# probcomp/GenParticleFilters.jl

Measured on AMD Instinct MI355X. Metric: particle-steps/sec, higher is better.
Workload: dtype f64; 1 GPU; 2D linear-Gaussian SSM, bootstrap PF, multinomial resample every step (BASELINE.json configs[1]); particles_per_gpu=1000000, particles_total=1000000, T=3059, state_dim=2, parallelism=particle-shard x1

## Files before the change

### genparticlefilters.jl_amd/csrc/gpf_host.hpp

```cpp
#pragma once
#include "../../include/gpf.h"
#include "gpf_kernels.hpp"

#include <hip/hip_ext.h>
#include <rccl/rccl.h>
#include <dlfcn.h>
#include <unistd.h>

#include <algorithm>
#include <cmath>
#include <cstdio>
#include <cstring>
#include <mutex>
#include <string>
#include <type_traits>
#include <vector>

using namespace gpf;

namespace gpfh {

static inline void cpu_relax()
{
#if defined(__x86_64__) || defined(__i386__)
// ... 54 lines not shown
    Scalars* sc = nullptr;
    Scalars* h_sc = nullptr;
    long long* h_sc_ticket = nullptr; long long sc_ticket = 0;
    uint32_t epoch = 0;
    bool initialized = false, has_prev = false, raw_valid = false, residual_scanned = false;
    bool max_valid = false;
    bool raw_sum_valid = false;
    WSum sum_cache{};
    uint64_t* sum_part = nullptr;
    int64_t* h_spart = nullptr;
    bool sum_on_host = false;
    uint64_t* gate_part = nullptr; int gate_cur = 0; int64_t* h_gate = nullptr;
    bool raw_has_q = false;
    bool raw_q_folded = false;
    bool pending_gather = false;
    bool pending_fill = false;
    bool pending_search = false;
    SearchArgs pend_sa{};
    bool pending_move = false; int pm_method = 0, pm_iters = 0; uint32_t pm_epoch = 0; ModelArgs pm_args{};
    bool lazy_move = true;
    bool lazy_search = false;
    bool want_offsets = true;
    bool ch0_offsets = false;
    bool offsets_hint = true;
    bool pending_packed = false;
    const double* pend_packed = nullptr; const double* pend_mf = nullptr; const int64_t* pend_tot = nullptr; int pend_G = 0;
    bool pend_mailbox = false;
    bool pend_own = false; int64_t pend_m = 0; bool pend_own_range = false;
    double* fuse_mf_out = nullptr;
    bool own_direct = false;
    bool own_direct_range = false;
    bool hist_on = false;
    int hist_cap = 0;
    std::vector<double*> hist_x;
    std::vector<int32_t*> hist_map;
    int hist_step = -1;
    const int32_t** hist_dev_maps = nullptr;
    gpf_filter* parent = nullptr;
    std::vector<gpf_filter*> views;
    bool orphaned = false;
    int64_t view_start = 0;
    int64_t view_step = 1;
    double* vrows[2] = {nullptr, nullptr}; double* vlw = nullptr; int32_t* vanc = nullptr;
    int32_t* vidx = nullptr; int32_t* vgid = nullptr;
    uint64_t generation = 0;
    uint64_t parent_generation = 0;
// ... 336 lines not shown
```

### genparticlefilters.jl_amd/csrc/gpf_k_scan.hpp

```cpp
#pragma once

namespace gpf {
static __global__ __launch_bounds__(BLOCK) void k_max_partial(PrioView pv, int64_t n, MaxSlots ms)
{
    double m = -__builtin_huge_val();
    int f = 0;
    for (int64_t i = (int64_t)blockIdx.x * BLOCK + threadIdx.x; i < n; i += (int64_t)gridDim.x * BLOCK) track_max(pv.at(i), m, f);
    block_max_store(m, f, ms);
}

constexpr uint64_t DESC_VALID = 1ull << 63, DESC_MASK = (1ull << 63) - 1;
constexpr unsigned SPIN_LIMIT = 1u << 22;

__device__ __forceinline__ void desc_store(uint64_t* p, uint64_t v)
{
    __hip_atomic_store(p, v, __ATOMIC_RELAXED, __HIP_MEMORY_SCOPE_AGENT);
}
__device__ __forceinline__ uint64_t desc_load(const uint64_t* p)
{
    return __hip_atomic_load(const_cast<uint64_t*>(p), __ATOMIC_RELAXED, __HIP_MEMORY_SCOPE_AGENT);
}
__device__ __forceinline__ uint64_t desc_wait(const uint64_t* p, int32_t* timeout)
{
    uint64_t d = desc_load(p);
// ... 104 lines not shown
};
#ifndef GPF_SCAN_BLOCK
#define GPF_SCAN_BLOCK 256
#endif
constexpr int SCAN_BLOCK = GPF_SCAN_BLOCK;
constexpr int SCAN_NWAVES = SCAN_BLOCK / WAVE;
constexpr int SCAN_ROWS = TILE / (2 * SCAN_BLOCK);
static_assert(SCAN_ROWS * 2 * SCAN_BLOCK == TILE && SCAN_ROWS >= 2 && SCAN_ROWS % 2 == 0, "a wave owns whole 256-element groups");
template <class In, int MODE>
__global__ __launch_bounds__(SCAN_BLOCK) void k_scan(In in, int64_t n, int64_t ntiles,
                                                const double* __restrict__ mf_all, const unsigned long long* __restrict__ slots,
                                                int np, WSum* __restrict__ ws_out, ScanOut out,
                                                uint64_t* __restrict__ dcur, uint64_t* __restrict__ dnext,
                                                uint64_t* __restrict__ total_out, uint64_t* __restrict__ blockQ,
                                                int32_t* __restrict__ timeout, ScanExtras ex)
{
    const unsigned G = gridDim.x - (unsigned)ex.sp.blocks;
    if (blockIdx.x >= G) { sorted_gamma_tile(ex.sp, (int64_t)(blockIdx.x - G) * SCAN_BLOCK + threadIdx.x); return; }
    if (ex.zero128 && blockIdx.x == 0)
        for (int i = threadIdx.x; i < 2 * MAX_SHARDS * ex.zero_stride; i += SCAN_BLOCK) ex.zero128[i] = 0;
    __shared__ uint64_t s_wave[SCAN_NWAVES];
    __shared__ uint64_t s_red[SCAN_NWAVES];
    __shared__ uint64_t s_Stot;
    uint64_t* const d_agg = dcur;
    uint64_t* const d_pre = dcur + ntiles;
    for (int64_t i = (int64_t)blockIdx.x * SCAN_BLOCK + threadIdx.x; i < 2 * ntiles; i += (int64_t)G * SCAN_BLOCK) dnext[i] = 0;
    constexpr bool WANT_Q = MODE == 2 || MODE == 4;
    double pre[2 * SCAN_ROWS];
    if constexpr (MODE >= 1) {
        const int64_t wb0 = (int64_t)blockIdx.x * TILE + (int64_t)wave_id() * (SCAN_ROWS * 2 * WAVE) + 2 * lane_id();
#pragma unroll
        for (int k = 0; k < SCAN_ROWS; ++k) in.raw2(wb0 + k * 2 * WAVE, n, pre[2 * k], pre[2 * k + 1]);
    }
    if constexpr (MODE >= 1) {
        double m; int f;
        if constexpr (MODE >= 3) {
            double m0 = 0.0; int f0 = 0;
            if (ex.fuse_mf) {
                fold_slots(slots, m0, f0);
                f0 &= FLAG_NAN | FLAG_POSINF;
                if (blockIdx.x == 0 && wave_id() == 0) {
                    if (lane_id() == 0) { ex.mf_out[0] = m0; ex.mf_out[1] = (double)f0; }
                    const uint64_t words[2] = {d2u(m0), d2u((double)f0)};
                    mbox_push_wave(ex.mf_push, words);
                }
            }
            mbox_wait_block(ex.wait);
            const int g = lane_id();
            const bool mb = ex.wait.tags != nullptr;
            const bool self = ex.fuse_mf && g == ex.mf_me;
            m = g < np ? (self ? m0 : ld_gathered(mf_all + 2 * g, mb)) : -__builtin_huge_val();
            f = g < np ? (self ? f0 : (int)ld_gathered(mf_all + 2 * g + 1, mb)) : 0;
            m = wave_max_f64(m);
#pragma unroll
            for (int s = 32; s >= 1; s >>= 1) f |= __shfl_xor(f, s, WAVE);
            if (!(f & FLAG_NAN) && m == -__builtin_huge_val()) f |= FLAG_ALL_NEGINF;
        } else fold_slots(slots, m, f);
        in.m = m; in.flags = f;
        if (blockIdx.x == 0 && threadIdx.x == 0) {
// ... 16 lines not shown
            uint64_t q0, q1;
            cb[k] = carry;
            if constexpr (MODE >= 1) {
                if (tile == blockIdx.x) in.conv2(wbase + k * 2 * WAVE, n, pre[2 * k], pre[2 * k + 1], q0, q1);
                else in.load2(wbase + k * 2 * WAVE, n, q0, q1);
            } else in.load2(wbase + k * 2 * WAVE, n, q0, q1);
            if constexpr (WANT_Q) {
                uint64_t lo = q0 * q0, hi = __umul64hi(q0, q0);
                ql[0] += lo & 0xffffffffull; ql[1] += lo >> 32; ql[2] += hi & 0xffffffffull; ql[3] += hi >> 32;
                lo = q1 * q1; hi = __umul64hi(q1, q1);
                ql[0] += lo & 0xffffffffull; ql[1] += lo >> 32; ql[2] += hi & 0xffffffffull; ql[3] += hi >> 32;
            }
            const uint64_t pair = q0 + q1;
            const uint64_t inc = wave_scan_u64(pair);
            p[2 * k] = carry + (inc - pair) + q0;
            p[2 * k + 1] = p[2 * k] + q1;
            carry += shfl_u64(inc, WAVE - 1);
        }
        if (lane == 0) s_wave[wv] = carry;
        __syncthreads();
        uint64_t wexcl = 0, agg = 0;
#pragma unroll
        for (int w = 0; w < SCAN_NWAVES; ++w) { if (w < wv) wexcl += s_wave[w]; agg += s_wave[w]; }
        if (threadIdx.x == 0) desc_store(d_agg + tile, DESC_VALID | agg);
        const int64_t first = (tile / G) * G;
        uint64_t acc = 0;
        for (int64_t idx = first + threadIdx.x; idx < tile; idx += SCAN_BLOCK) acc += desc_wait(d_agg + idx, timeout);
        if (first > 0 && threadIdx.x == SCAN_BLOCK - 1) acc += desc_wait(d_pre + first - 1, timeout);
        acc = wave_sum_u64(acc);
        if (lane == 0) s_red[wv] = acc;
        __syncthreads();
        uint64_t excl = 0;
#pragma unroll
        for (int w = 0; w < SCAN_NWAVES; ++w) excl += s_red[w];
        if (threadIdx.x == 0) desc_store(d_pre + tile, DESC_VALID | (excl + agg));
        const uint64_t off = excl + wexcl;
        if (out.cdf) {
#pragma unroll
            for (int k = 0; k < SCAN_ROWS; ++k) {
                const int64_t idx = wbase + k * 2 * WAVE;
                const uint64_t v1 = off + p[2 * k + 1];
                *reinterpret_cast<ulonglong2*>(out.cdf + idx) = make_ulonglong2(off + p[2 * k], v1);
                if ((lane & 7) == 7) out.t16[(idx + 1) >> 4] = v1;
                if ((lane & 15) == 15) out.k32[(idx + 1) >> 5] = (uint32_t)(key_sat(v1) >> KEY_SHIFT);
                if (lane == WAVE - 1 && (k & 1)) out.t256[(idx + 1) >> 8] = v1;
                if (out.k32s && lane == WAVE - 1) out.k32s[(idx + 1) >> 7] = (uint32_t)(key_sat(v1) >> KEY_SHIFT);
                if (out.off16) {
                    const int GL = 16 << out.logg;
                    const uint32_t kv = (uint32_t)(key_sat(v1) >> KEY_SHIFT);
                    const uint32_t khi = (uint32_t)__shfl((int)kv, lane | (GL - 1), WAVE);
                    const uint32_t kprev = (uint32_t)__shfl((int)kv, ((lane & ~(GL - 1)) - 1) & (WAVE - 1), WAVE);
                    const uint32_t klo = lane < GL ? (uint32_t)(key_sat(off + cb[k]) >> KEY_SHIFT) : kprev;
                    const int sh = key_quant_shift(klo, khi);
                    const uint64_t kb = (uint64_t)klo << KEY_SHIFT;
                    const uint32_t o0 = (uint32_t)((key_sat(off + p[2 * k]) - kb) >> sh), o1 = (uint32_t)((key_sat(v1) - kb) >> sh);
                    reinterpret_cast<uint32_t*>(out.off16)[idx >> 1] = o0 | (o1 << 16);
                    if (out.logg == 0) {
                        const uint32_t part = (uint32_t)__builtin_amdgcn_update_dpp(0, (int)o1, 0x55, 0xF, 0xF, false);
                        if ((lane & 3) == 3) reinterpret_cast<uint32_t*>(out.coarse)[(idx + 1) >> 3] = part | (o1 << 16);
                    } else {
                        const uint32_t part = (uint32_t)__builtin_amdgcn_update_dpp(0, (int)o1, 0x114, 0xF, 0xF, false);
                        if ((lane & 7) == 7) reinterpret_cast<uint32_t*>(out.coarse)[(idx + 1) >> 4] = part | (o1 << 16);
                    }
                }
            }
        }
        if constexpr (MODE == 3) {
            if (tile == ntiles - 1 && wv == SCAN_NWAVES - 1) {
                const uint64_t Sw = shfl_u64(off + p[2 * SCAN_ROWS - 1], WAVE - 1);
                const uint64_t words[5] = {Sw, 0, 0, 0, 0};
                mbox_push_wave(ex.push, words);
            }
        }
        if (tile == ntiles - 1 && threadIdx.x == SCAN_BLOCK - 1) {
            const uint64_t Stot = off + p[2 * SCAN_ROWS - 1];
            *total_out = Stot;
            if constexpr (WANT_Q) s_Stot = Stot;
            if constexpr (MODE >= 1) {
                if (ex.n_slots > 0) {
                    const uint64_t Bq = Stot / (uint64_t)ex.n_slots;
                    ws_out->sB = Bq; ws_out->srem = Stot - Bq * (uint64_t)ex.n_slots;
                    ws_out->sinv = (double)ex.n_slots / (double)Stot;
                }
            }
        }
        if constexpr (MODE == 3) {
            if (ex.splan.plan && tile == ntiles - 1) {
                static_assert(SCAN_BLOCK > MAX_SHARDS, "one thread per shard boundary");
                __shared__ int64_t s_F[MAX_SHARDS + 1];
                const StratPlanJob& jb = ex.splan;
                strat_plan_body(jb, [&](int g) { return shard_bound(jb.n_global, jb.G, g); }, s_F);
            }
        }
        __syncthreads();
    }
    if constexpr (WANT_Q) {
        __shared__ uint64_t s_q[SCAN_NWAVES][4];
// ... 522 lines not shown
```

### genparticlefilters.jl_amd/csrc/gpf_k_search.hpp

```cpp
#pragma once

namespace gpf {
struct CdfLevels {
    const uint64_t* cdf;  const uint64_t* t16;  const uint64_t* t256;  const uint64_t* ttile;
    const uint32_t* k32;
    const uint16_t* off16; const uint16_t* coarse; int logg;
    const uint32_t* k32s; int sample;
};
__device__ __forceinline__ ulonglong2 load_global_16(uint64_t addr, int sub)
{
#if defined(__HIP_DEVICE_COMPILE__)
    typedef unsigned long long __attribute__((ext_vector_type(2))) u64x2;
    const __attribute__((address_space(1))) u64x2* g = reinterpret_cast<const __attribute__((address_space(1))) u64x2*>(addr);
    const u64x2 v = g[sub];
    return make_ulonglong2(v.x, v.y);
#else
    (void)addr; (void)sub;
    return make_ulonglong2(0, 0);
#endif
}

__device__ __forceinline__ int group8_sum(int c)
{
    c += __builtin_amdgcn_update_dpp(0, c, 0xB1, 0xF, 0xF, false);
    c += __builtin_amdgcn_update_dpp(0, c, 0x4E, 0xF, 0xF, false);
    c += __builtin_amdgcn_update_dpp(0, c, 0x141, 0xF, 0xF, false);
    return c;
}
__device__ __forceinline__ void coop_count_le2(const uint64_t* line0, uint64_t T0, const uint64_t* line1, uint64_t T1,
                                               ulonglong2* lds_wave, int& c0, int& c1)
// ... 240 lines not shown
            head[u] = false; top[u] = st.topw; L[u] = &a.w;
            if (METHOD == 0) T[u] = mulhi64(U, S);
            else if (METHOD == 3) {
                T[u] = jg * s_div[0] + (jg * s_div[1] + mulhi64(U, S)) / N;
            } else {
                head[u] = jg < Ctot;
                T[u] = head[u] ? jg : mulhi64(U, S);
                if (head[u]) { top[u] = st.topc; L[u] = &a.c; }
            }
        }
        const bool coop = METHOD == 0 ? true : (METHOD == 3 ? false : __any(!head[0] || !head[1]) != 0);
        int64_t idx[2];
        search_pair(st, L, top, T, coop, lds_wave, a.n_cells, a.ntiles, idx);
#pragma unroll
        for (int u = 0; u < 2; ++u) {
            if (act[u]) a.anc[j[u]] = (int32_t)idx[u];
        }
    }
}

constexpr int MULTI_LDS_BUDGET = 160 * 1024 - 2048;
__host__ __device__ __forceinline__ int64_t multi_groups(int64_t ntiles, int logg) { return (ntiles * (TILE / 32)) >> logg; }
__host__ __device__ __forceinline__ uint32_t kpad(uint32_t i) { return i + (i >> 5); }
__host__ inline size_t multi_lds_bytes(int64_t ntiles, int logg) { return (size_t)(kpad((uint32_t)multi_groups(ntiles, logg)) + 1) * sizeof(uint32_t); }
#ifndef GPF_MULTI_MIN_LOGG
#define GPF_MULTI_MIN_LOGG 0
#endif
__host__ inline int multi_logg(int64_t ntiles)
{
    for (int g = GPF_MULTI_MIN_LOGG; g <= 1; ++g) if (multi_lds_bytes(ntiles, g) <= (size_t)MULTI_LDS_BUDGET) return g;
    return -1;
}
constexpr int MULTI_SAMPLE_MAX = 2;
__host__ inline int multi_sample(int64_t ntiles)
{
    if (multi_logg(ntiles) >= 0) return 0;
    for (int s = 2; s <= MULTI_SAMPLE_MAX; ++s) if (multi_lds_bytes(ntiles, s) <= (size_t)MULTI_LDS_BUDGET) return s;
    return 0;
}
typedef unsigned short __attribute__((ext_vector_type(2))) u16x2;
__device__ __forceinline__ uint32_t pk_lt(uint32_t x, uint32_t qq)
{
    const u16x2 d = __builtin_elementwise_sub_sat(__builtin_bit_cast(u16x2, qq), __builtin_bit_cast(u16x2, x));
    const u16x2 one = {1, 1};
    return __builtin_bit_cast(uint32_t, __builtin_elementwise_min(d, one));
}
__device__ __forceinline__ uint32_t pk_ne(uint32_t x, uint32_t qq)
// ... 328 lines not shown
                const Philox b = rng(a.seed, sb + (uint32_t)q, 0, a.epoch, TAG_RESAMPLE);
                if (q > 0) T[2 * q - 1] = mulhi64(u64(b.w0, b.w1), S);
                if (q < NS / 2) T[2 * q] = mulhi64(u64(b.w2, b.w3), S);
            }
        }
    };
    const int64_t stride = (int64_t)gridDim.x * NS * SBLOCK;
    int64_t base = (int64_t)blockIdx.x * NS * SBLOCK;
    uint64_t T[NS];
    const MultiTable tb = multi_table_load<LOGG>(a.w, a.ntiles, S, reinterpret_cast<uint32_t*>(smem), [&]() { targets(base, T); });
    for (; base < a.n; base += stride) {
        const int64_t j0 = base + NS * (int64_t)threadIdx.x;
        uint32_t idx[NS];
        multi_lookup<LOGG, NS>(tb, a.w, a.n_cells, T, idx);
        int32_t* dst = a.anc + j0;
        if (j0 + NS <= a.n && (reinterpret_cast<uintptr_t>(dst) & (4 * NS - 1)) == 0) {
            if (NS == 4) *reinterpret_cast<int4*>(dst) = make_int4((int32_t)idx[0], (int32_t)idx[1], (int32_t)idx[2], (int32_t)idx[3]);
            else *reinterpret_cast<int2*>(dst) = make_int2((int32_t)idx[0], (int32_t)idx[1]);
        } else {
#pragma unroll
            for (int u = 0; u < NS; ++u) if (j0 + u < a.n) dst[u] = (int32_t)idx[u];
        }
        if (base + stride < a.n) targets(base + stride, T);
    }
}

constexpr int MBLOCK = 256;
#ifndef GPF_MSLOTS
#define GPF_MSLOTS 8
#endif
constexpr int MSLOTS = GPF_MSLOTS;
constexpr int MJB = MBLOCK * MSLOTS;
#ifndef GPF_MONO_WIDE_MULT
#define GPF_MONO_WIDE_MULT 2
#endif
#ifndef GPF_MONO_WIDE2_MULT
#define GPF_MONO_WIDE2_MULT 64
#endif
#ifndef GPF_WIDE_NS
#define GPF_WIDE_NS 4
#endif
constexpr int MONO_WIDE_NS = GPF_WIDE_NS;
constexpr int64_t MONO_WIDE = GPF_MONO_WIDE_MULT * (int64_t)MJB;
constexpr int64_t MONO_WIDE2 = GPF_MONO_WIDE2_MULT * (int64_t)MJB;

template <class Between>
// ... 508 lines not shown
```

### genparticlefilters.jl_amd/csrc/libgpf_aux.hip

```cpp
#include "gpf_host.hpp"
#include "gpf_k_coalesce.hpp"

using namespace gpf;
using namespace gpfh;

namespace gpfh {

template <int M, int MODE, bool BP>
void launch_init_blk(gpf_filter* h, int grid)
{
    if constexpr (MODE == 2 && !Model<M>::HAS_STRATA) { (void)h; (void)grid; return; }
    else GPF_LAUNCH((k_init<M, MODE, true, BP>), dim3(grid), dim3(BLOCK), 0, h->stream, h->args, h->cfg.seed, h->epoch,
                    h->cfg.gid0, h->n, h->W, h->rows[h->cur], h->lw, next_slots(h));
}
template <int M, int MODE, bool KEEP, bool BP>
void launch_step_blk(gpf_filter* h, int grid)
{
    constexpr int Wc = row_width(Model<M>::D, KEEP);
    if constexpr ((MODE == 2 && !Model<M>::HAS_STRATA) || (MODE == 4 && !Model<M>::HAS_PROPOSAL)) { (void)h; (void)grid; return; }
    else GPF_LAUNCH((k_step<M, Wc, KEEP, false, MODE, false, true, BP>), dim3(grid), dim3(BLOCK), 0, h->stream, h->args, h->cfg.seed, h->epoch,
                    h->cfg.gid0, h->n, h->anc, h->rows[h->cur], h->rows[1 - h->cur], h->lw, next_slots(h), PackedCommit{});
}
template <int M, bool RW, bool BP>
void launch_move_blk(gpf_filter* h, int grid, int n_iters)
// ... 1118 lines not shown
    for (int i = 0; same && i < hd.n_params; ++i) same = memcmp(&hd.params[i], &h->args.P[i], sizeof(double)) == 0;
    if (!same) return fail(h, GPF_ERR_INVALID_ARGUMENT, "the checkpoint was taken of a filter with another gpf_config (model, parameters, particle counts, gid0, seed, keep_prev)");
    if (bytes != ckpt_bytes(h)) return fail(h, GPF_ERR_INVALID_ARGUMENT, "truncated checkpoint");
    if (h->hist_on) return fail(h, GPF_ERR_STATE, "a filter with a trajectory store cannot load a checkpoint (the store is not part of it)");
    HIP_TRY(h, hipSetDevice(h->cfg.device));
    for (gpf_filter* v : h->blk_views) gpf_destroy(v);
    h->blk_views.clear();
    h->pending_move = false; h->pending_search = false; h->pending_gather = false; h->pending_fill = false;
    h->pending_packed = false; h->pend_ring = false;
    const char* o = static_cast<const char*>(in) + sizeof(CkptHeader);
    const size_t rb = (size_t)h->n * h->W * 8, wb = (size_t)h->n * 8, ab = (size_t)h->n * 4;
    HIP_TRY(h, hipMemcpyAsync(h->rows[h->cur], o, rb, hipMemcpyHostToDevice, h->stream));
    HIP_TRY(h, hipMemcpyAsync(h->lw, o + rb, wb, hipMemcpyHostToDevice, h->stream));
    HIP_TRY(h, hipMemcpyAsync(h->anc, o + rb + wb, ab, hipMemcpyHostToDevice, h->stream));
    HIP_TRY(h, hipMemcpyAsync(reinterpret_cast<char*>(h->sc) + offsetof(Scalars, lml_est), &hd.lml_est, sizeof(double), hipMemcpyHostToDevice, h->stream));
    HIP_TRY(h, hipStreamSynchronize(h->stream));
    h->epoch = hd.epoch; h->has_prev = hd.has_prev != 0; h->initialized = true;
    h->args.n_strata = hd.n_strata; h->args.interleaved = hd.interleaved; h->args.logK = hd.logK;
    for (int i = 0; i < MAX_OBS; ++i) h->args.obs[i] = hd.obs[i];
    for (int i = 0; i < MAX_STRATA; ++i) h->args.strata[i] = hd.strata[i];
    for (int i = 0; i < 4; ++i) h->args.q[i] = hd.q[i];
    h->blk_obs_size = 0;
    h->raw_valid = false; h->raw_sum_valid = false; h->max_valid = false; h->raw_has_q = false; h->raw_q_folded = false;
    h->residual_scanned = false; h->push_counted = false; h->gsum_ok = false; h->ch0_offsets = false;
    mutated(h);
    return GPF_OK;
}

gpf_status gpf_history_mean(gpf_handle h, int32_t step, int32_t column, double* out) { return history_stat(h, step, column, out, false); }
gpf_status gpf_history_var(gpf_handle h, int32_t step, int32_t column, double* out) { return history_stat(h, step, column, out, true); }


}
```

### genparticlefilters.jl_amd/csrc/libgpf_resample.hip

```cpp
#include "gpf_host.hpp"

using namespace gpf;
using namespace gpfh;

namespace gpfh {

template <class In, int FIXQ>
gpf_status scan_launch(gpf_filter* h, int ch, const In& in, int np, WSum* slot, bool want_cdf, uint64_t* total_out,
                       const double* mf_all = nullptr, ScanExtras ex = ScanExtras{nullptr, nullptr, 0, 0})
{
    uint64_t* dc = h->desc[ch][h->dcur[ch]];
    uint64_t* dn = h->desc[ch][1 - h->dcur[ch]];
    int gs = std::is_same<In, InFixQ>::value ? wscan_grid(h) : scan_grid(h);
    if (h->sp_job_set && std::is_same<In, InFixQ>::value) { ex.sp = h->sp_job; ex.sp.blocks = (int)((h->sp_job.ntl + SCAN_BLOCK - 1) / SCAN_BLOCK); h->sp_job_set = false; }
    const int g_launch = gs + ex.sp.blocks;
    const bool offsets = ch == 0 && h->want_offsets && want_cdf;
    const ScanOut so = scan_out(want_cdf ? h->cdf[ch] : nullptr, h->t16[ch], h->t256[ch], h->ntiles, offsets);
    if (ch == 0 && want_cdf) h->ch0_offsets = offsets && so.off16 != nullptr;
    const ChainScope chain(h);
    gpf_status s = timed(h, GPF_K_SCAN, [&] {
        GPF_LAUNCH((k_scan<In, FIXQ>), dim3(g_launch), dim3(SCAN_BLOCK), 0, h->stream, in, h->n, h->ntiles, mf_all, h->mslots[h->mcur], np, slot,
                           so, dc, dn, total_out, h->blockQ, h->h_timeout, ex);
    });
    if (s) return s;
    h->table[ch] = dc + h->ntiles;
    h->dcur[ch] ^= 1;
    return GPF_OK;
}

gpf_status scan_launch_shard(gpf_filter* h, int mode, const InFixQ& in, int np, WSum* slot, bool want_cdf, uint64_t* total_out, const double* mf_all, const ScanExtras& ex)
{
    return mode == 4 ? scan_launch<InFixQ, 4>(h, 0, in, np, slot, want_cdf, total_out, mf_all, ex) : scan_launch<InFixQ, 3>(h, 0, in, np, slot, want_cdf, total_out, mf_all, ex);
}
gpf_status scan_launch_optimal(gpf_filter* h, int ch, const InOptimal& in, uint64_t* total_out)
{
    return scan_launch<InOptimal, 0>(h, ch, in, 0, nullptr, true, total_out);
}

gpf_status resample_device_setup(gpf_filter* h)
{
        {
// ... 5 lines not shown
            for (const void* f : scans) {
                int q = 0;
                HIP_TRY(h, hipOccupancyMaxActiveBlocksPerMultiprocessor(&q, f, SCAN_BLOCK, 0));
                if (q < 1) return fail(h, GPF_ERR_HIP, "a scan kernel cannot be resident on this device");
                nb = std::min(nb, q > 2 ? q - 1 : q);
            }
            h->scan_blocks_per_cu = std::max(1, std::min(nb, 2));
            int wb = 64;
            for (int k = 0; k < 4; ++k) {
                int q = 0;
                HIP_TRY(h, hipOccupancyMaxActiveBlocksPerMultiprocessor(&q, scans[k], SCAN_BLOCK, 0));
                wb = std::min(wb, q > 2 ? q - 1 : q);
            }
            static const int wscan_max = getenv("GPF_WSCAN_BLOCKS") ? atoi(getenv("GPF_WSCAN_BLOCKS")) : 4;
            h->wscan_blocks_per_cu = std::max(1, std::min(std::min(wb, wscan_max), 8));
        }
        const int max_dyn = (int)((lds_pad(LDS_TILE_TABLE) + 4) * sizeof(uint64_t));
        HIP_TRY(h, hipFuncSetAttribute(reinterpret_cast<const void*>(&k_search<0>), hipFuncAttributeMaxDynamicSharedMemorySize, max_dyn));
        HIP_TRY(h, hipFuncSetAttribute(reinterpret_cast<const void*>(&k_search<1>), hipFuncAttributeMaxDynamicSharedMemorySize, max_dyn));
        HIP_TRY(h, hipFuncSetAttribute(reinterpret_cast<const void*>(&k_search<3>), hipFuncAttributeMaxDynamicSharedMemorySize, max_dyn));
        HIP_TRY(h, hipFuncSetAttribute(reinterpret_cast<const void*>(&k_search_multi<0>), hipFuncAttributeMaxDynamicSharedMemorySize, MULTI_LDS_BUDGET));
        HIP_TRY(h, hipFuncSetAttribute(reinterpret_cast<const void*>(&k_search_multi<1>), hipFuncAttributeMaxDynamicSharedMemorySize, MULTI_LDS_BUDGET));
        HIP_TRY(h, hipFuncSetAttribute(reinterpret_cast<const void*>(&k_search_multi_s<2>), hipFuncAttributeMaxDynamicSharedMemorySize, MULTI_LDS_BUDGET));
    return GPF_OK;
}

gpf_status ensure_max(gpf_filter* h, const PrioView& pv, bool use_producer_max)
{
    if (use_producer_max && h->max_valid) return GPF_OK;
    const int gp = (int)std::min<int64_t>(MAX_PARTIALS, (h->n + BLOCK - 1) / BLOCK);
    gpf_status s = timed(h, GPF_K_MAX, [&] {
        GPF_LAUNCH(k_max_partial, dim3(gp), dim3(BLOCK), 0, h->stream, pv, h->n, next_slots(h));
    });
    if (s) return s;
    h->max_valid = use_producer_max;
    return GPF_OK;
}
gpf_status summarize(gpf_filter* h, const PrioView& pv, WSum* slot, bool want_cdf, const int32_t* order, bool use_producer_max,
                     bool want_q, bool publish_flags, bool max_ready)
{
    ScanExtras ex{nullptr, nullptr, 0, h->cfg.n_global};
    if (publish_flags) {
        if (!h->h_flags) { HIP_TRY(h, hipHostMalloc(&h->h_flags, 2 * sizeof(int64_t))); h->h_flags[0] = h->h_flags[1] = 0; }
        h->flag_ticket += 1;
        ex.host_flags = h->h_flags; ex.ticket = h->flag_ticket;
    }
// ... 379 lines not shown
    bool pending = false, flagged = false;
    gpf_status s = sort_desc_begin(h, pv, n, &pending);
    if (s || !pending) return s;
    if ((s = sort_desc_flagged(h, &flagged))) return s;
    return flagged ? sort_passes(h, pv, n, false) : GPF_OK;
}

gpf_status ensure_residual_buffers(gpf_filter* h)
{
    for (int i = 1; i < 3; ++i) {
        if (h->cdf[i]) continue;
        HIP_TRY(h, hipMalloc(&h->cdf[i], (size_t)h->ntiles * TILE * sizeof(uint64_t)));
        HIP_TRY(h, hipMalloc(&h->t16[i], (size_t)h->ntiles * (TILE / 16) * sizeof(uint64_t)));
        HIP_TRY(h, hipMalloc(&h->t256[i], t256_bytes(h->ntiles)));
    }
    return GPF_OK;
}

CdfLevels levels(const gpf_filter* h, int ch)
{
    int logg = ch == 0 && h->ch0_offsets ? multi_logg(h->ntiles) : -1;
    const int sample = ch == 0 && h->ch0_offsets && logg < 0 ? multi_sample(h->ntiles) : 0;
    if (sample > 0) logg = 0;
    return CdfLevels{h->cdf[ch], h->t16[ch], h->t256[ch], h->table[ch], k32_of(h->t256[ch], h->ntiles),
                     logg >= 0 ? off16_of(h->t256[ch], h->ntiles) : nullptr, logg >= 0 ? coarse_of(h->t256[ch], h->ntiles) : nullptr, logg,
                     sample > 0 ? k32s_of(h->t256[ch], h->ntiles) : nullptr, sample};
}

gpf_status residual_scans(gpf_filter* h, const WSum* ws, int64_t n_slots_global, int32_t* head_anc, const ResidDirect* direct)
{
    gpf_status s = ensure_residual_buffers(h);
    if (s) return s;
    Scan2Chan ch[2];
    for (int c = 0; c < 2; ++c) {
        const int id = 1 + c;
        uint64_t* dc = h->desc[id][h->dcur[id]];
        ch[c].out = scan_out(h->cdf[id], h->t16[id], h->t256[id], h->ntiles, false);
        ch[c].dcur = dc; ch[c].dnext = h->desc[id][1 - h->dcur[id]];
        ch[c].total_out = c == 0 ? &h->sc->Ctot : &h->sc->Rs;
        h->table[id] = dc + h->ntiles;
        h->dcur[id] ^= 1;
    }
    const int gs = scan_grid(h);
    const ChainScope chain(h);
    s = timed(h, GPF_K_SCAN, [&] {
        if (direct) GPF_LAUNCH(k_scan_residual2<true>, dim3(gs), dim3(SCAN_BLOCK), 0, h->stream, h->cdf[0], ws, n_slots_global, h->n, h->ntiles, ch[0], ch[1], h->h_timeout, head_anc, &h->sc->giants, h->epoch & 0xffffffu, *direct);
        else        GPF_LAUNCH(k_scan_residual2<false>, dim3(gs), dim3(SCAN_BLOCK), 0, h->stream, h->cdf[0], ws, n_slots_global, h->n, h->ntiles, ch[0], ch[1], h->h_timeout, head_anc, &h->sc->giants, h->epoch & 0xffffffu, ResidDirect{});
    });
    if (s) return s;
    HIP_TRY(h, hipGetLastError());
    return GPF_OK;
}

void launch_multinomial_search(gpf_filter* h, const SearchArgs& sa)
{
    const int logg = sa.w.off16 && sa.w.sample == 0 ? sa.w.logg : -1;
    if (sa.w.off16 && sa.w.sample > 0) {
        const int gss = (int)std::max<int64_t>(1, std::min<int64_t>((sa.n + 2 * SBLOCK - 1) / (2 * SBLOCK), (int64_t)h->n_cu));
        const size_t lds = multi_lds_bytes(sa.ntiles, sa.w.sample);
        static_assert(MULTI_SAMPLE_MAX == 2, "one instantiation");
        GPF_LAUNCH((k_search_multi_s<2>), dim3(gss), dim3(SBLOCK), lds, h->stream, sa);
        return;
    }
    const int gsr = (int)std::max<int64_t>(1, std::min<int64_t>((sa.n + 2 * SBLOCK - 1) / (2 * SBLOCK), (int64_t)h->n_cu));
    if (logg == 0)      GPF_LAUNCH((k_search_multi<0>), dim3(gsr), dim3(SBLOCK), multi_lds_bytes(sa.ntiles, 0), h->stream, sa);
    else if (logg == 1) GPF_LAUNCH((k_search_multi<1>), dim3(gsr), dim3(SBLOCK), multi_lds_bytes(sa.ntiles, 1), h->stream, sa);
    else                GPF_LAUNCH((k_search<0>), dim3(gsr), dim3(SBLOCK), search_lds_bytes(sa.ntiles, 1), h->stream, sa);
}

void launch_search_plain(gpf_filter* h, int which, int grid, size_t lds, const SearchArgs& sa)
{
    if (which == 1) GPF_LAUNCH((k_search<1>), dim3(grid), dim3(SBLOCK), lds, h->stream, sa);
    else            GPF_LAUNCH((k_search<3>), dim3(grid), dim3(SBLOCK), lds, h->stream, sa);
}
void launch_search_strat(gpf_filter* h, const SearchArgs& sa, int64_t n_slots, bool sorted_uniforms)
{
    if (sorted_uniforms) GPF_LAUNCH((k_search_strat<true>), dim3((unsigned)((n_slots + MJB - 1) / MJB)), dim3(MBLOCK), 0, h->stream, sa);
    else                 GPF_LAUNCH((k_search_strat<false>), dim3((unsigned)((n_slots + MJB_STRAT - 1) / MJB_STRAT)), dim3(MBLOCK), 0, h->stream, sa);
}
gpf_status sorted_job_prepare(gpf_filter* h, int64_t gid0, int64_t n_slots)
{
    const int64_t ntl = (n_slots + SP_TILE - 1) / SP_TILE;
    if (h->sp_cap < ntl + 1) {
        if (h->sp_g) { HIP_TRY(h, hipStreamSynchronize(h->stream)); (void)hipFree(h->sp_g); (void)hipFree(h->sp_vlo); h->sp_g = h->sp_vlo = nullptr; h->sp_cap = 0; }
        HIP_TRY(h, hipMalloc(&h->sp_g, (size_t)(ntl + 1) * sizeof(uint64_t)));
        HIP_TRY(h, hipMalloc(&h->sp_vlo, (size_t)(ntl + 1) * sizeof(uint64_t)));
        h->sp_cap = ntl + 1;
// ... 20 lines not shown
    h->pending_search = false;
    gpf_status s = timed(h, GPF_K_SEARCH, [&] { launch_multinomial_search(h, h->pend_sa); });
    if (s) return s;
    HIP_TRY(h, hipGetLastError());
    return GPF_OK;
}
bool lazy_search_ok(const gpf_filter* h)
{
    const bool off = !h->lazy_search;
    const int logg = multi_logg(h->ntiles);
    return !off && !h->parent && !h->hist_on && h->cfg.n_global == h->n && logg >= 0 &&
           multi_lds_bytes(h->ntiles, logg) + 16 + FUSED_LDS_EXTRA + 1024 <= (size_t)160 * 1024;
}

gpf_status resample_impl(gpf_filter* h, int method, PrioView pv, int sort_particles, int check, int32_t* invalid, bool local)
{
    if (method != GPF_RESAMPLE_MULTINOMIAL && method != GPF_RESAMPLE_RESIDUAL && method != GPF_RESAMPLE_STRATIFIED && method != GPF_RESAMPLE_MULTINOMIAL_SORTED)
        return fail(h, GPF_ERR_UNKNOWN_METHOD, "Resampling method not recognized.");
    if (h->cfg.n_global != h->n)
        return fail(h, GPF_ERR_STATE, "sharded filters resample through the shard-level API (sharded.py)");
    const bool sorted = method == GPF_RESAMPLE_STRATIFIED && sort_particles;
    const bool need_sync = check == GPF_CHECK_TRUE || invalid != nullptr;
    const bool need_off = method == GPF_RESAMPLE_MULTINOMIAL && (multi_logg(h->ntiles) >= 0 || multi_sample(h->ntiles) > 0);
    struct OffScope { gpf_filter* h; ~OffScope() { h->want_offsets = true; } } off_scope{h};
    h->want_offsets = need_off;
    h->offsets_hint = need_off;
    gpf_status s;
    if ((s = check_scan_timeout(h))) return s;
    if ((s = materialize(h))) return s;
    if (pv.mode != 0 && (s = ensure_raw(h))) return s;
    bool sort_pending = false;
    if (sorted) {
        if ((s = ensure_max(h, pv, pv.mode == 0))) return s;
        if ((s = sort_desc_begin(h, pv, h->n, &sort_pending))) return s;
    }
    if (method == GPF_RESAMPLE_MULTINOMIAL_SORTED) {
        if ((s = sorted_job_prepare(h, h->cfg.gid0, h->n))) return s;
    }
    struct SpScope { gpf_filter* h; ~SpScope() { h->sp_job_set = false; } } sp_scope{h};
    WSum* ws;
    bool published = false;
    static const bool no_direct = getenv("GPF_RESIDUAL_DIRECT") && !strcmp(getenv("GPF_RESIDUAL_DIRECT"), "0");
    ResidDirect rdirect{};
    const bool resid_direct = !no_direct && method == GPF_RESAMPLE_RESIDUAL && pv.mode == 0 && !h->raw_valid && h->raw_sum_valid && h->sum_on_host;
    int direct_flags = 0;
    if (resid_direct) {
        rdirect = ResidDirect{h->lw, h->sum_cache.m, h->sum_cache.flags, h->K, h->sum_cache.S, &h->sc->raw, nullptr, 0, 0};
        direct_flags = h->sum_cache.flags;
        ws = &h->sc->raw;
    } else
    if (pv.mode == 0) {
        ws = &h->sc->raw;
        if (!h->raw_valid || sorted || (need_off && !h->ch0_offsets)) {
            if ((s = summarize(h, pv, ws, true, sorted ? h->order : nullptr, true, false, need_sync, sorted))) return s;
            published = need_sync;
        }
    } else {
        h->want_offsets = need_off;
        ws = &h->sc->prio;
        if ((s = summarize(h, pv, ws, true, sorted ? h->order : nullptr, false, false, need_sync, sorted))) return s;
        published = need_sync;
    }
    h->raw_valid = false; h->raw_sum_valid = false;
    h->raw_q_folded = false;
    if (need_sync) {
        int flags;
        if (published) {
            if ((s = wait_ticket(h, h->h_flags + 1, h->flag_ticket, "weight scan flags"))) return s;
            flags = (int)h->h_flags[0];
        } else if (resid_direct) flags = direct_flags;
        else {
            if ((s = fetch_scalars(h))) return s;
            flags = (pv.mode == 0 ? h->h_sc->raw : h->h_sc->prio).flags;
        }
        const bool inv = flags != 0;
        h->last_flags = flags;
        if (invalid) *invalid = inv ? 1 : 0;
        if (flags & (FLAG_NAN | FLAG_POSINF)) return fail(h, GPF_ERR_INVALID_WEIGHTS, "Invalid weights (NaN).");
        if (check == GPF_CHECK_TRUE && inv) return fail(h, GPF_ERR_INVALID_WEIGHTS, "Invalid weights.");
    }
    SearchArgs sa{};
    sa.w = levels(h, 0); sa.c = levels(h, 0); sa.ntiles = h->ntiles;
    sa.order = sorted ? h->order : nullptr; sa.sc = h->sc; sa.ws = ws; sa.raw = &h->sc->raw; sa.n = h->n; sa.n_cells = h->n;
// ... 217 lines not shown
```

Before: 20.24 billion particle-steps/sec.

## Add local-scan mode that skips decoupled lookback and rebuilds tile offsets in search

Adds a scan mode (MODE 5) that writes only per-tile aggregates and skips the decoupled-lookback chain, the dnext zeroing, the t256/k32s writes and the total store. A new multinomial search kernel loads the aggregates into LDS, prefix-sums them per block to rebuild tile offsets and the total, then locates each draw with a windowed local search. The aim is to remove the cross-block serialization in the scan, in exchange for redundant per-block aggregate scans in search and extra LDS use. It applies only when lazy search is not possible and the tile count fits the per-lane aggregate budget.

```diff
diff --git a/genparticlefilters.jl_amd/csrc/gpf_host.hpp b/genparticlefilters.jl_amd/csrc/gpf_host.hpp
--- a/genparticlefilters.jl_amd/csrc/gpf_host.hpp
+++ b/genparticlefilters.jl_amd/csrc/gpf_host.hpp
@@ -100,6 +100,8 @@
     bool lazy_search = false;
     bool want_offsets = true;
     bool ch0_offsets = false;
+    bool want_local = false;
+    bool ch0_local = false;
     bool offsets_hint = true;
     bool pending_packed = false;
     const double* pend_packed = nullptr; const double* pend_mf = nullptr; const int64_t* pend_tot = nullptr; int pend_G = 0;
diff --git a/genparticlefilters.jl_amd/csrc/gpf_k_scan.hpp b/genparticlefilters.jl_amd/csrc/gpf_k_scan.hpp
--- a/genparticlefilters.jl_amd/csrc/gpf_k_scan.hpp
+++ b/genparticlefilters.jl_amd/csrc/gpf_k_scan.hpp
@@ -150,9 +150,11 @@
     __shared__ uint64_t s_wave[SCAN_NWAVES];
     __shared__ uint64_t s_red[SCAN_NWAVES];
     __shared__ uint64_t s_Stot;
+    constexpr bool LOCAL = MODE == 5, SHARD = MODE == 3 || MODE == 4;
     uint64_t* const d_agg = dcur;
     uint64_t* const d_pre = dcur + ntiles;
-    for (int64_t i = (int64_t)blockIdx.x * SCAN_BLOCK + threadIdx.x; i < 2 * ntiles; i += (int64_t)G * SCAN_BLOCK) dnext[i] = 0;
+    if constexpr (!LOCAL)
+        for (int64_t i = (int64_t)blockIdx.x * SCAN_BLOCK + threadIdx.x; i < 2 * ntiles; i += (int64_t)G * SCAN_BLOCK) dnext[i] = 0;
     constexpr bool WANT_Q = MODE == 2 || MODE == 4;
     double pre[2 * SCAN_ROWS];
     if constexpr (MODE >= 1) {
@@ -162,7 +164,7 @@
     }
     if constexpr (MODE >= 1) {
         double m; int f;
-        if constexpr (MODE >= 3) {
+        if constexpr (SHARD) {
             double m0 = 0.0; int f0 = 0;
             if (ex.fuse_mf) {
                 fold_slots(slots, m0, f0);
@@ -225,18 +227,22 @@
         uint64_t wexcl = 0, agg = 0;
 #pragma unroll
         for (int w = 0; w < SCAN_NWAVES; ++w) { if (w < wv) wexcl += s_wave[w]; agg += s_wave[w]; }
-        if (threadIdx.x == 0) desc_store(d_agg + tile, DESC_VALID | agg);
-        const int64_t first = (tile / G) * G;
-        uint64_t acc = 0;
-        for (int64_t idx = first + threadIdx.x; idx < tile; idx += SCAN_BLOCK) acc += desc_wait(d_agg + idx, timeout);
-        if (first > 0 && threadIdx.x == SCAN_BLOCK - 1) acc += desc_wait(d_pre + first - 1, timeout);
-        acc = wave_sum_u64(acc);
-        if (lane == 0) s_red[wv] = acc;
-        __syncthreads();
         uint64_t excl = 0;
-#pragma unroll
-        for (int w = 0; w < SCAN_NWAVES; ++w) excl += s_red[w];
-        if (threadIdx.x == 0) desc_store(d_pre + tile, DESC_VALID | (excl + agg));
+        if constexpr (LOCAL) {
+            if (threadIdx.x == 0) d_agg[tile] = agg;
+        } else {
+            if (threadIdx.x == 0) desc_store(d_agg + tile, DESC_VALID | agg);
+            const int64_t first = (tile / G) * G;
+            uint64_t acc = 0;
+            for (int64_t idx = first + threadIdx.x; idx < tile; idx += SCAN_BLOCK) acc += desc_wait(d_agg + idx, timeout);
+            if (first > 0 && threadIdx.x == SCAN_BLOCK - 1) acc += desc_wait(d_pre + first - 1, timeout);
+            acc = wave_sum_u64(acc);
+            if (lane == 0) s_red[wv] = acc;
+            __syncthreads();
+#pragma unroll
+            for (int w = 0; w < SCAN_NWAVES; ++w) excl += s_red[w];
+            if (threadIdx.x == 0) desc_store(d_pre + tile, DESC_VALID | (excl + agg));
+        }
         const uint64_t off = excl + wexcl;
         if (out.cdf) {
 #pragma unroll
@@ -246,8 +252,8 @@
                 *reinterpret_cast<ulonglong2*>(out.cdf + idx) = make_ulonglong2(off + p[2 * k], v1);
                 if ((lane & 7) == 7) out.t16[(idx + 1) >> 4] = v1;
                 if ((lane & 15) == 15) out.k32[(idx + 1) >> 5] = (uint32_t)(key_sat(v1) >> KEY_SHIFT);
-                if (lane == WAVE - 1 && (k & 1)) out.t256[(idx + 1) >> 8] = v1;
-                if (out.k32s && lane == WAVE - 1) out.k32s[(idx + 1) >> 7] = (uint32_t)(key_sat(v1) >> KEY_SHIFT);
+                if constexpr (!LOCAL) if (lane == WAVE - 1 && (k & 1)) out.t256[(idx + 1) >> 8] = v1;
+                if constexpr (!LOCAL) if (out.k32s && lane == WAVE - 1) out.k32s[(idx + 1) >> 7] = (uint32_t)(key_sat(v1) >> KEY_SHIFT);
                 if (out.off16) {
                     const int GL = 16 << out.logg;
                     const uint32_t kv = (uint32_t)(key_sat(v1) >> KEY_SHIFT);
@@ -275,7 +281,7 @@
                 mbox_push_wave(ex.push, words);
             }
         }
-        if (tile == ntiles - 1 && threadIdx.x == SCAN_BLOCK - 1) {
+        if constexpr (!LOCAL) if (tile == ntiles - 1 && threadIdx.x == SCAN_BLOCK - 1) {
             const uint64_t Stot = off + p[2 * SCAN_ROWS - 1];
             *total_out = Stot;
             if constexpr (WANT_Q) s_Stot = Stot;
diff --git a/genparticlefilters.jl_amd/csrc/gpf_k_search.hpp b/genparticlefilters.jl_amd/csrc/gpf_k_search.hpp
--- a/genparticlefilters.jl_amd/csrc/gpf_k_search.hpp
+++ b/genparticlefilters.jl_amd/csrc/gpf_k_search.hpp
@@ -6,6 +6,7 @@
     const uint32_t* k32;
     const uint16_t* off16; const uint16_t* coarse; int logg;
     const uint32_t* k32s; int sample;
+    const uint64_t* agg;
 };
 __device__ __forceinline__ ulonglong2 load_global_16(uint64_t addr, int sub)
 {
@@ -292,7 +293,8 @@
 constexpr int MULTI_LDS_BUDGET = 160 * 1024 - 2048;
 __host__ __device__ __forceinline__ int64_t multi_groups(int64_t ntiles, int logg) { return (ntiles * (TILE / 32)) >> logg; }
 __host__ __device__ __forceinline__ uint32_t kpad(uint32_t i) { return i + (i >> 5); }
-__host__ inline size_t multi_lds_bytes(int64_t ntiles, int logg) { return (size_t)(kpad((uint32_t)multi_groups(ntiles, logg)) + 1) * sizeof(uint32_t); }
+__host__ __device__ __forceinline__ size_t multi_keys_bytes(int64_t ntiles, int logg) { return ((size_t)(kpad((uint32_t)multi_groups(ntiles, logg)) + 1) * sizeof(uint32_t) + 7) & ~(size_t)7; }
+__host__ inline size_t multi_lds_bytes(int64_t ntiles, int logg) { return multi_keys_bytes(ntiles, logg) + (size_t)(ntiles + 1) * sizeof(uint64_t); }
 #ifndef GPF_MULTI_MIN_LOGG
 #define GPF_MULTI_MIN_LOGG 0
 #endif
@@ -667,6 +669,184 @@
             for (int u = 0; u < NS; ++u) if (j0 + u < a.n) dst[u] = (int32_t)idx[u];
         }
         if (base + stride < a.n) targets(base + stride, T);
+    }
+}
+
+constexpr uint32_t LOCAL_WIN = 8;
+constexpr int LOCAL_AGG_PER_LANE = 2;
+struct LocalTable { const uint32_t* keys; const uint64_t* O; uint32_t nt, p2; float tscale; };
+template <int LOGG, int NS>
+__device__ __forceinline__ void multi_lookup_local(const LocalTable& tb, const CdfLevels& w, int64_t n_cells, const uint64_t (&T)[NS], uint32_t (&idx)[NS])
+{
+    constexpr uint32_t KPT = (TILE / 32) >> LOGG;
+    constexpr int G = 32 << LOGG;
+    uint32_t tile[NS];
+    bool inwin = tb.nt >= LOCAL_WIN;
+#pragma unroll
+    for (int u = 0; u < NS; ++u) {
+        const uint32_t pe = (uint32_t)((float)(uint32_t)(T[u] >> KEY_SHIFT) * tb.tscale);
+        uint32_t lo = pe > LOCAL_WIN / 2 ? pe - LOCAL_WIN / 2 : 0u;
+        lo = lo + LOCAL_WIN > tb.nt ? tb.nt - LOCAL_WIN : lo;
+        tile[u] = lo;
+    }
+    if (inwin) {
+#pragma unroll
+        for (int u = 0; u < NS; ++u) inwin = inwin && tb.O[tile[u]] <= T[u] && T[u] < tb.O[tile[u] + LOCAL_WIN];
+    }
+    if (__all(inwin)) {
+#pragma unroll
+        for (uint32_t h = LOCAL_WIN / 2; h >= 1; h >>= 1) {
+#pragma unroll
+            for (int u = 0; u < NS; ++u) tile[u] += tb.O[tile[u] + h] <= T[u] ? h : 0u;
+        }
+    } else {
+#pragma unroll
+        for (int u = 0; u < NS; ++u) tile[u] = tb.O[tb.p2] <= T[u] ? tb.nt - tb.p2 : 0u;
+        for (uint32_t h = tb.p2 >> 1; h >= 1; h >>= 1) {
+#pragma unroll
+            for (int u = 0; u < NS; ++u) tile[u] += tb.O[tile[u] + h] <= T[u] ? h : 0u;
+        }
+#pragma unroll
+        for (int u = 0; u < NS; ++u) {
+            tile[u] += tb.O[tile[u] + 1] <= T[u] ? 1u : 0u;
+            tile[u] = tile[u] < tb.nt ? tile[u] : tb.nt - 1;
+        }
+    }
+    uint64_t Tl[NS]; uint32_t t[NS], base[NS], pos[NS];
+#pragma unroll
+    for (int u = 0; u < NS; ++u) {
+        const uint64_t o = tb.O[tile[u]];
+        Tl[u] = T[u] >= o ? T[u] - o : 0;
+        t[u] = (uint32_t)(Tl[u] >> KEY_SHIFT);
+        base[u] = tile[u] * KPT;
+        pos[u] = 0;
+    }
+#pragma unroll
+    for (uint32_t h = KPT / 2; h >= 1; h >>= 1) {
+#pragma unroll
+        for (int u = 0; u < NS; ++u) pos[u] += tb.keys[kpad(base[u] + pos[u] + h - 1)] < t[u] ? h : 0u;
+    }
+    bool amb = false;
+#pragma unroll
+    for (int u = 0; u < NS; ++u) {
+        pos[u] += tb.keys[kpad(base[u] + pos[u])] < t[u] ? 1u : 0u;
+        pos[u] = pos[u] < KPT ? pos[u] : KPT - 1;
+        amb = amb || tb.keys[kpad(base[u] + pos[u])] == t[u];
+    }
+    if (__any(amb)) {
+#pragma unroll
+        for (int u = 0; u < NS; ++u) {
+            if (tb.keys[kpad(base[u] + pos[u])] != t[u]) continue;
+            uint32_t lo = pos[u], hi;
+            {
+                uint32_t a = lo + 1, b = KPT;
+                while (a < b) { const uint32_t mid = (a + b) >> 1; if (tb.keys[kpad(base[u] + mid)] <= t[u]) a = mid + 1; else b = mid; }
+                hi = a;
+            }
+            while (lo < hi) {
+                const uint32_t mid = (lo + hi) >> 1;
+                if (w.cdf[(int64_t)(base[u] + mid) * G + (G - 1)] <= Tl[u]) lo = mid + 1; else hi = mid;
+            }
+            pos[u] = lo < KPT ? lo : KPT - 1;
+        }
+    }
+    uint32_t g[NS], klo[NS], khi[NS];
+#pragma unroll
+    for (int u = 0; u < NS; ++u) {
+        g[u] = base[u] + pos[u];
+        klo[u] = pos[u] ? tb.keys[kpad(g[u] - 1)] : 0u; khi[u] = tb.keys[kpad(g[u])];
+    }
+    multi_inside_k<LOGG, NS>(g, klo, khi, w, n_cells, Tl, idx);
+}
+
+template <int LOGG>
+__global__ __launch_bounds__(SBLOCK, 4) void k_search_multi_local(SearchArgs a)
+{
+    constexpr int NS = GPF_MULTI_NS;
+    constexpr int NW = SBLOCK / WAVE;
+    constexpr int KT = (MULTI_LDS_BUDGET / 4 / (LOGG == 0 ? 4 : 2) + SBLOCK - 1) / SBLOCK;
+    static_assert(LOCAL_AGG_PER_LANE == 2, "one 16-byte load of aggregates per lane");
+    extern __shared__ __attribute__((aligned(16))) unsigned char smem[];
+    __shared__ uint64_t s_wtot[NW];
+    uint32_t* const keys = reinterpret_cast<uint32_t*>(smem);
+    uint64_t* const O = reinterpret_cast<uint64_t*>(smem + multi_keys_bytes(a.ntiles, LOGG));
+    LocalTable tb;
+    tb.keys = keys; tb.O = O; tb.nt = (uint32_t)a.ntiles;
+    const uint32_t ng = (uint32_t)multi_groups(a.ntiles, LOGG);
+    const uint32_t nq = LOGG == 0 ? ng / 4 : ng / 2;
+    uint4 kv[KT];
+    const uint4* src = reinterpret_cast<const uint4*>(a.w.k32);
+#pragma unroll
+    for (int r = 0; r < KT; ++r) { const uint32_t q = threadIdx.x + (uint32_t)r * SBLOCK; if (q < nq) kv[r] = src[q]; }
+    const uint32_t t0 = 2 * threadIdx.x;
+    const uint64_t a0 = t0 < tb.nt ? a.w.agg[t0] : 0, a1 = t0 + 1 < tb.nt ? a.w.agg[t0 + 1] : 0;
+    auto draws = [&](int64_t base, uint64_t* U) {
+        const uint32_t s0 = (uint32_t)(a.gid0 + base + NS * (int64_t)threadIdx.x), sb = s0 >> 1;
+        if (!(s0 & 1u)) {
+#pragma unroll
+            for (int q = 0; q < NS / 2; ++q) {
+                const Philox b = rng(a.seed, sb + (uint32_t)q, 0, a.epoch, TAG_RESAMPLE);
+                U[2 * q] = u64(b.w0, b.w1); U[2 * q + 1] = u64(b.w2, b.w3);
+            }
+        } else {
+#pragma unroll
+            for (int q = 0; q <= NS / 2; ++q) {
+                const Philox b = rng(a.seed, sb + (uint32_t)q, 0, a.epoch, TAG_RESAMPLE);
+                if (q > 0) U[2 * q - 1] = u64(b.w0, b.w1);
+                if (q < NS / 2) U[2 * q] = u64(b.w2, b.w3);
+            }
+        }
+    };
+    const int64_t stride = (int64_t)gridDim.x * NS * SBLOCK;
+    int64_t base = (int64_t)blockIdx.x * NS * SBLOCK;
+    uint64_t T[NS];
+    draws(base, T);
+    tb.p2 = 1;
+    while (2 * tb.p2 <= tb.nt) tb.p2 *= 2;
+    const uint64_t pair = a0 + a1;
+    const uint64_t inc = wave_scan_u64(pair);
+    if (lane_id() == WAVE - 1) s_wtot[wave_id()] = inc;
+    __syncthreads();
+    uint64_t wexcl = 0, S = 0;
+#pragma unroll
+    for (int w = 0; w < NW; ++w) { const uint64_t v = s_wtot[w]; if (w < (int)wave_id()) wexcl += v; S += v; }
+    const uint64_t excl = wexcl + (inc - pair);
+    if (threadIdx.x == 0) O[0] = 0;
+    if (t0 < tb.nt) O[t0 + 1] = excl + a0;
+    if (t0 + 1 < tb.nt) O[t0 + 2] = excl + pair;
+    if (blockIdx.x == 0 && threadIdx.x == 0) {
+        const_cast<WSum*>(a.ws)->S = S;
+        if (a.update_lml) resample_bookkeeping(a);
+    }
+    tb.tscale = (float)tb.nt / (float)((S >> KEY_SHIFT) + 1);
+#pragma unroll
+    for (int u = 0; u < NS; ++u) T[u] = mulhi64(T[u], S);
+#pragma unroll
+    for (int r = 0; r < KT; ++r) {
+        const uint32_t q = threadIdx.x + (uint32_t)r * SBLOCK;
+        if (q < nq) {
+            if (LOGG == 0) { uint32_t* d = keys + kpad(4 * q); d[0] = kv[r].x; d[1] = kv[r].y; d[2] = kv[r].z; d[3] = kv[r].w; }
+            else { uint32_t* d = keys + kpad(2 * q); d[0] = kv[r].y; d[1] = kv[r].w; }
+        }
+    }
+    __syncthreads();
+    for (; base < a.n; base += stride) {
+        const int64_t j0 = base + NS * (int64_t)threadIdx.x;
+        uint32_t idx[NS];
+        multi_lookup_local<LOGG, NS>(tb, a.w, a.n_cells, T, idx);
+        int32_t* dst = a.anc + j0;
+        if (j0 + NS <= a.n && (reinterpret_cast<uintptr_t>(dst) & (4 * NS - 1)) == 0) {
+            if (NS == 4) *reinterpret_cast<int4*>(dst) = make_int4((int32_t)idx[0], (int32_t)idx[1], (int32_t)idx[2], (int32_t)idx[3]);
+            else *reinterpret_cast<int2*>(dst) = make_int2((int32_t)idx[0], (int32_t)idx[1]);
+        } else {
+#pragma unroll
+            for (int u = 0; u < NS; ++u) if (j0 + u < a.n) dst[u] = (int32_t)idx[u];
+        }
+        if (base + stride < a.n) {
+            draws(base + stride, T);
+#pragma unroll
+            for (int u = 0; u < NS; ++u) T[u] = mulhi64(T[u], S);
+        }
     }
 }
 
diff --git a/genparticlefilters.jl_amd/csrc/libgpf_aux.hip b/genparticlefilters.jl_amd/csrc/libgpf_aux.hip
--- a/genparticlefilters.jl_amd/csrc/libgpf_aux.hip
+++ b/genparticlefilters.jl_amd/csrc/libgpf_aux.hip
@@ -1164,7 +1164,7 @@
     for (int i = 0; i < 4; ++i) h->args.q[i] = hd.q[i];
     h->blk_obs_size = 0;
     h->raw_valid = false; h->raw_sum_valid = false; h->max_valid = false; h->raw_has_q = false; h->raw_q_folded = false;
-    h->residual_scanned = false; h->push_counted = false; h->gsum_ok = false; h->ch0_offsets = false;
+    h->residual_scanned = false; h->push_counted = false; h->gsum_ok = false; h->ch0_offsets = false; h->ch0_local = false;
     mutated(h);
     return GPF_OK;
 }
diff --git a/genparticlefilters.jl_amd/csrc/libgpf_resample.hip b/genparticlefilters.jl_amd/csrc/libgpf_resample.hip
--- a/genparticlefilters.jl_amd/csrc/libgpf_resample.hip
+++ b/genparticlefilters.jl_amd/csrc/libgpf_resample.hip
@@ -17,6 +17,19 @@
     const bool offsets = ch == 0 && h->want_offsets && want_cdf;
     const ScanOut so = scan_out(want_cdf ? h->cdf[ch] : nullptr, h->t16[ch], h->t256[ch], h->ntiles, offsets);
     if (ch == 0 && want_cdf) h->ch0_offsets = offsets && so.off16 != nullptr;
+    if constexpr (std::is_same<In, InFixQ>::value && FIXQ == 1) {
+        if (ch == 0 && h->want_local && want_cdf && so.off16 != nullptr && so.sample == 0 && h->ntiles <= (int64_t)LOCAL_AGG_PER_LANE * SBLOCK) {
+            gpf_status sl = timed(h, GPF_K_SCAN, [&] {
+                GPF_LAUNCH((k_scan<InFixQ, 5>), dim3(g_launch), dim3(SCAN_BLOCK), 0, h->stream, in, h->n, h->ntiles, mf_all, h->mslots[h->mcur], np, slot,
+                                   so, h->t256[0], static_cast<uint64_t*>(nullptr), static_cast<uint64_t*>(nullptr), h->blockQ, static_cast<int32_t*>(nullptr), ex);
+            });
+            if (sl) return sl;
+            h->ch0_local = true;
+            h->table[0] = nullptr;
+            return GPF_OK;
+        }
+    }
+    if (ch == 0 && want_cdf) h->ch0_local = false;
     const ChainScope chain(h);
     gpf_status s = timed(h, GPF_K_SCAN, [&] {
         GPF_LAUNCH((k_scan<In, FIXQ>), dim3(g_launch), dim3(SCAN_BLOCK), 0, h->stream, in, h->n, h->ntiles, mf_all, h->mslots[h->mcur], np, slot,
@@ -68,6 +81,8 @@
         HIP_TRY(h, hipFuncSetAttribute(reinterpret_cast<const void*>(&k_search_multi<0>), hipFuncAttributeMaxDynamicSharedMemorySize, MULTI_LDS_BUDGET));
         HIP_TRY(h, hipFuncSetAttribute(reinterpret_cast<const void*>(&k_search_multi<1>), hipFuncAttributeMaxDynamicSharedMemorySize, MULTI_LDS_BUDGET));
         HIP_TRY(h, hipFuncSetAttribute(reinterpret_cast<const void*>(&k_search_multi_s<2>), hipFuncAttributeMaxDynamicSharedMemorySize, MULTI_LDS_BUDGET));
+        HIP_TRY(h, hipFuncSetAttribute(reinterpret_cast<const void*>(&k_search_multi_local<0>), hipFuncAttributeMaxDynamicSharedMemorySize, MULTI_LDS_BUDGET));
+        HIP_TRY(h, hipFuncSetAttribute(reinterpret_cast<const void*>(&k_search_multi_local<1>), hipFuncAttributeMaxDynamicSharedMemorySize, MULTI_LDS_BUDGET));
     return GPF_OK;
 }
 
@@ -493,9 +508,12 @@
     int logg = ch == 0 && h->ch0_offsets ? multi_logg(h->ntiles) : -1;
     const int sample = ch == 0 && h->ch0_offsets && logg < 0 ? multi_sample(h->ntiles) : 0;
     if (sample > 0) logg = 0;
+    if (ch == 0 && h->ch0_local)
+        return CdfLevels{h->cdf[0], h->t16[0], nullptr, nullptr, k32_of(h->t256[0], h->ntiles), off16_of(h->t256[0], h->ntiles), coarse_of(h->t256[0], h->ntiles), logg,
+                         nullptr, 0, h->t256[0]};
     return CdfLevels{h->cdf[ch], h->t16[ch], h->t256[ch], h->table[ch], k32_of(h->t256[ch], h->ntiles),
                      logg >= 0 ? off16_of(h->t256[ch], h->ntiles) : nullptr, logg >= 0 ? coarse_of(h->t256[ch], h->ntiles) : nullptr, logg,
-                     sample > 0 ? k32s_of(h->t256[ch], h->ntiles) : nullptr, sample};
+                     sample > 0 ? k32s_of(h->t256[ch], h->ntiles) : nullptr, sample, nullptr};
 }
 
 gpf_status residual_scans(gpf_filter* h, const WSum* ws, int64_t n_slots_global, int32_t* head_anc, const ResidDirect* direct)
@@ -534,6 +552,11 @@
         return;
     }
     const int gsr = (int)std::max<int64_t>(1, std::min<int64_t>((sa.n + 2 * SBLOCK - 1) / (2 * SBLOCK), (int64_t)h->n_cu));
+    if (sa.w.agg) {
+        if (logg == 0) GPF_LAUNCH((k_search_multi_local<0>), dim3(gsr), dim3(SBLOCK), multi_lds_bytes(sa.ntiles, 0), h->stream, sa);
+        else           GPF_LAUNCH((k_search_multi_local<1>), dim3(gsr), dim3(SBLOCK), multi_lds_bytes(sa.ntiles, 1), h->stream, sa);
+        return;
+    }
     if (logg == 0)      GPF_LAUNCH((k_search_multi<0>), dim3(gsr), dim3(SBLOCK), multi_lds_bytes(sa.ntiles, 0), h->stream, sa);
     else if (logg == 1) GPF_LAUNCH((k_search_multi<1>), dim3(gsr), dim3(SBLOCK), multi_lds_bytes(sa.ntiles, 1), h->stream, sa);
     else                GPF_LAUNCH((k_search<0>), dim3(gsr), dim3(SBLOCK), search_lds_bytes(sa.ntiles, 1), h->stream, sa);
@@ -600,9 +623,12 @@
     const bool sorted = method == GPF_RESAMPLE_STRATIFIED && sort_particles;
     const bool need_sync = check == GPF_CHECK_TRUE || invalid != nullptr;
     const bool need_off = method == GPF_RESAMPLE_MULTINOMIAL && (multi_logg(h->ntiles) >= 0 || multi_sample(h->ntiles) > 0);
-    struct OffScope { gpf_filter* h; ~OffScope() { h->want_offsets = true; } } off_scope{h};
+    struct OffScope { gpf_filter* h; ~OffScope() { h->want_offsets = true; h->want_local = false; } } off_scope{h};
     h->want_offsets = need_off;
     h->offsets_hint = need_off;
+    static const bool local_off = getenv("GPF_SCAN_LOCAL") && !strcmp(getenv("GPF_SCAN_LOCAL"), "0");
+    const bool lazy_possible = pv.mode == 0 && !local && lazy_search_ok(h);
+    const bool scan_local = !local_off && method == GPF_RESAMPLE_MULTINOMIAL && multi_logg(h->ntiles) >= 0 && !lazy_possible;
     gpf_status s;
     if ((s = check_scan_timeout(h))) return s;
     if ((s = materialize(h))) return s;
@@ -630,13 +656,19 @@
     if (pv.mode == 0) {
         ws = &h->sc->raw;
         if (!h->raw_valid || sorted || (need_off && !h->ch0_offsets)) {
-            if ((s = summarize(h, pv, ws, true, sorted ? h->order : nullptr, true, false, need_sync, sorted))) return s;
+            h->want_local = scan_local;
+            s = summarize(h, pv, ws, true, sorted ? h->order : nullptr, true, false, need_sync, sorted);
+            h->want_local = false;
+            if (s) return s;
             published = need_sync;
         }
     } else {
         h->want_offsets = need_off;
         ws = &h->sc->prio;
-        if ((s = summarize(h, pv, ws, true, sorted ? h->order : nullptr, false, false, need_sync, sorted))) return s;
+        h->want_local = scan_local;
+        s = summarize(h, pv, ws, true, sorted ? h->order : nullptr, false, false, need_sync, sorted);
+        h->want_local = false;
+        if (s) return s;
         published = need_sync;
     }
     h->raw_valid = false; h->raw_sum_valid = false;
```

After: 19.70 billion particle-steps/sec. 2.6% lower.
